# nabeelscicom/DistilCodec_nabeel

Measured on AMD Instinct MI355X. Metric: 24 kHz samples/s encode+decode at 1/8 GPU; code-index bit-exact vs CPU, higher is better.
Workload: dtype f32

## Files before the change

### distilcodec_nabeel_amd/csrc/dcx_conv_common.h

```cpp
#pragma once
#include <algorithm>
#include <type_traits>

#include "dcx_kernels.h"
#include "dcx_planes.h"

namespace dcx {

typedef float f32x16 __attribute__((ext_vector_type(16)));
typedef float f32x4 __attribute__((ext_vector_type(4)));
typedef float f32x2 __attribute__((ext_vector_type(2)));
typedef short s16x8 __attribute__((ext_vector_type(8)));
typedef short s16x4 __attribute__((ext_vector_type(4)));
typedef __bf16 bf16x8 __attribute__((ext_vector_type(8)));

constexpr int BK = 16;
constexpr int LDSK = 20;
template <bool SWZ>
struct XRow {
  static constexpr int kStride = SWZ ? 48 : 56;
  __device__ static __forceinline__ int half(int row, int h) { return SWZ ? h ^ ((row >> 3) & 1) : h; }
  __device__ static __forceinline__ int off(int row, int piece) {
    const int h = piece >= 3;
    return row * kStride + (half(row, h) * 3 + piece - 3 * h) * 8;
  }
};

__device__ __forceinline__ float silu_f(float v) { return v * __builtin_amdgcn_rcpf(1.0f + __expf(-v)); }
__device__ __forceinline__ float gelu_f(float v) { return 0.5f * v * (1.0f + erff(v * 0.70710678118654752440f)); }
__device__ __forceinline__ float gelu_bf16_f(float v) {
#ifdef DCX_GELU_ERF
  return gelu_f(v);
#endif
  const float z = fabsf(v) * 0.70710678118654752440f;
  const float t = __builtin_amdgcn_rcpf(fmaf(0.5f, z, 1.0f));
  float q = 0.17087277f;
  q = fmaf(q, t, -0.82215223f);
  q = fmaf(q, t, 1.48851587f);
  q = fmaf(q, t, -1.13520398f);
  q = fmaf(q, t, 0.27886807f);
  q = fmaf(q, t, -0.18628806f);
  q = fmaf(q, t, 0.09678418f);
  q = fmaf(q, t, 0.37409196f);
  q = fmaf(q, t, 1.00002368f);
  const float c = t * __expf(fmaf(t, q, fmaf(-z, z, -1.26551223f)));
  const float e = v >= 0.0f ? 1.0f - c : c - 1.0f;
  return 0.5f * v * (1.0f + e);
}

__device__ __forceinline__ f32x2 gelu_bf16_f2(f32x2 v) {
#ifdef DCX_GELU_SCALAR
  return f32x2{gelu_bf16_f(v[0]), gelu_bf16_f(v[1])};
#endif
  const f32x2 z = __builtin_elementwise_abs(v) * 0.70710678118654752440f;
  const f32x2 d = __builtin_elementwise_fma(f32x2{0.5f, 0.5f}, z, f32x2{1.0f, 1.0f});
  const f32x2 t = {__builtin_amdgcn_rcpf(d[0]), __builtin_amdgcn_rcpf(d[1])};
  auto fm = [&](f32x2 q, float c) { return __builtin_elementwise_fma(q, t, f32x2{c, c}); };
  f32x2 q = {0.17087277f, 0.17087277f};
  q = fm(q, -0.82215223f);
  q = fm(q, 1.48851587f);
  q = fm(q, -1.13520398f);
  q = fm(q, 0.27886807f);
  q = fm(q, -0.18628806f);
  q = fm(q, 0.09678418f);
  q = fm(q, 0.37409196f);
  q = fm(q, 1.00002368f);
  const f32x2 arg = __builtin_elementwise_fma(t, q, __builtin_elementwise_fma(-z, z, f32x2{-1.26551223f, -1.26551223f}));
  const f32x2 c = t * f32x2{__expf(arg[0]), __expf(arg[1])};
  const f32x2 e = {v[0] >= 0.0f ? 1.0f - c[0] : c[0] - 1.0f, v[1] >= 0.0f ? 1.0f - c[1] : c[1] - 1.0f};
  return 0.5f * v * (1.0f + e);
}

__device__ __forceinline__ int xcd_remap(int bid, int nwg) {
  const int xcd = bid & 7, q = nwg >> 3, r = nwg & 7;
  return (xcd < r ? xcd * (q + 1) : r * (q + 1) + (xcd - r) * q) + (bid >> 3);
}

__device__ __forceinline__ void flat_tile(int tpc, int batch, int& wg, int& b, int& ph) {
  const int t = xcd_remap(blockIdx.x, gridDim.x);
  const int per_ph = tpc * batch;
  ph = t / per_ph;
  const int r = t - ph * per_ph;
  b = r / tpc;
  wg = r - b * tpc;
}

__device__ __forceinline__ void ksplit_slice(const ConvParams& p, int b, int& clip, int& c0, int& nchunks) {
  clip = b;
  c0 = 0;
  nchunks = p.Cin / BK;
  if (p.ksplit > 1) {
    const int clips = p.batch / p.ksplit, sl = b / clips;
    clip = b - sl * clips;
    const int nunits = nchunks / p.kunit, base = nunits / p.ksplit, extra = nunits % p.ksplit;
    c0 = (sl * base + min(sl, extra)) * p.kunit;
    nchunks = (base + (sl < extra ? 1 : 0)) * p.kunit;
  }
}

static __device__ __attribute__((used, aligned(16))) float g_zero_row[32] = {0.f};

#if defined(DCX_CLOCK_DIAG) || defined(DCX_SEG_DIAG) || defined(DCX_TILE_DIAG)
#define DCX_DIAG 1
constexpr int kTileDiagMax = 16384;
[[maybe_unused]] static __device__ unsigned long long g_clock_diag[3], g_seg_diag[13], g_seg_diag8[49];
[[maybe_unused]] static __device__ unsigned long long g_tile_diag[kTileDiagMax * 6];
[[maybe_unused]] static __device__ unsigned int g_tile_cnt;
enum DiagSet : int { DIAG_CLOCK, DIAG_SEG, DIAG_SEG8, DIAG_TILES };
static int diag_read(int set, unsigned long long* out, int n, int reset) {
  if (set == DIAG_TILES) {
    unsigned int cnt = 0;
    if (hipMemcpyFromSymbol(&cnt, HIP_SYMBOL(g_tile_cnt), sizeof cnt) != hipSuccess) return -1;
    cnt = std::min(cnt, (unsigned)std::max(0, std::min(n, kTileDiagMax)));
    if (cnt && hipMemcpyFromSymbol(out, HIP_SYMBOL(g_tile_diag), sizeof(unsigned long long) * 6 * cnt) != hipSuccess) return -1;
    const unsigned int z = 0;
    if (reset && hipMemcpyToSymbol(HIP_SYMBOL(g_tile_cnt), &z, sizeof z) != hipSuccess) return -1;
    return (int)cnt;
  }
  const void* sym = set == DIAG_CLOCK ? (const void*)g_clock_diag : set == DIAG_SEG ? (const void*)g_seg_diag : (const void*)g_seg_diag8;
  unsigned long long v[49] = {};
  if (n > 49 || hipMemcpyFromSymbol(v, sym, sizeof(unsigned long long) * n) != hipSuccess) return -1;
  for (int i = 0; i < n; ++i) out[i] += v[i];
  const unsigned long long z[49] = {};
  if (reset && hipMemcpyToSymbol(sym, z, sizeof(unsigned long long) * n) != hipSuccess) return -1;
  return 0;
}
#define DCX_DIAG_FILE(tag) \
  int diag_##tag(int set, unsigned long long* out, int n, int reset) { return diag_read(set, out, n, reset); }
#else
#define DCX_DIAG_FILE(tag)
#endif
#ifdef DCX_SEG_DIAG
#define DCX_SEGT(v) const unsigned long long v = __builtin_amdgcn_s_memtime()
#else
#define DCX_SEGT(v)
#endif
#ifdef DCX_TILE_DIAG
#define DCX_TILET(v) const unsigned long long v = __builtin_amdgcn_s_memrealtime()
#else
#define DCX_TILET(v)
#endif

struct EpiPre {
  int osh;
  float acur;
  bool track;
};
template <int RROW>
__device__ __forceinline__ EpiPre epi_range_pre(const ConvParams& p, const ConvParams& pr, int b) {
  EpiPre e{0, 0.f, false};
  const bool h2o = (p.y6 && p.y_layout == LAYOUT_H2) || (p.y6s && p.ys_layout != LAYOUT_PLANES);
  const bool h2row = (RROW & 2) && h2o && pr.yb.rowwise;
  if (h2o && !h2row) {
    const float bnd = range_bound(pr.yb, b);
    e.osh = __builtin_amdgcn_readfirstlane(h2_shift(bnd));
    if (threadIdx.x == 0) {
      if (pr.y_ash) pr.y_ash[b] = e.osh;
      if (pr.rflag && !(bnd <= 3.0e38f)) atomicOr(pr.rflag, RANGE_NONFINITE);
    }
  }
  const bool track = pr.y_amax != nullptr;
  e.track = track;
  e.acur = track && !h2row ? __builtin_bit_cast(float, __builtin_amdgcn_readfirstlane(
                                                           __builtin_bit_cast(int, range_cur(pr.y_amax, b))))
                           : 0.f;
  return e;
}

struct EpiGeneric {
  static constexpr bool fixed = false;
};
template <int EPI, int MEAN, bool Y, bool Y2, bool Y6H, bool Y6SH, bool TRACK, bool ROWWISE = false>
struct EpiForm {
  static constexpr bool fixed = true;
  static constexpr int epi = EPI, mean = MEAN;
  static constexpr bool y = Y, y2 = Y2, y6h = Y6H, y6sh = Y6SH, track = TRACK, rowwise = ROWWISE;
};
template <typename F>
inline bool epi_form_is(const ConvParams& p) {
  const bool h2o = F::y6h || F::y6sh;
  return p.epi == F::epi && p.mean_mode == F::mean && !p.round_bf16 && (p.y != nullptr) == F::y &&
         (p.y2 != nullptr) == F::y2 && (p.y6 != nullptr) == F::y6h && (p.y6s != nullptr) == F::y6sh &&
         (!p.y6 || p.y_layout == LAYOUT_H2) && (!p.y6s || p.ys_layout == LAYOUT_H2) && (p.y_amax != nullptr) == F::track &&
         (h2o ? (p.yb.rowwise != 0) == F::rowwise : true) && (F::epi != EPI_GELU || p.w6 != nullptr) &&
         (F::mean == MEAN_NONE || p.macc != nullptr);
}

template <int BM, int BN, int WM, int WN, int LDS_FLOATS, int NT, int RROW, bool RAG, typename F, typename AccT>
__device__ __forceinline__ void epilogue_form(const ConvParams& p, const ConvParams& pr, AccT& acc, int q0, int co0, int b,
                                              int ph, float* smem, const EpiPre& pre) {
  constexpr int WR = BM / WM, WC = BN / WN;
  static_assert(sizeof(acc[0][0]) == 16 && sizeof(acc) == WR * WC * 4 / 64, "16 x 16 accumulator blocks");
  constexpr int LDSW = BN + 4;
  constexpr int RPP = (BM * LDSW <= LDS_FLOATS) ? BM
                      : (BM / 2 * LDSW <= LDS_FLOATS) ? BM / 2
                      : (BM / 4 * LDSW <= LDS_FLOATS) ? BM / 4 : WR;
  static_assert(RPP % WR == 0 && RPP * LDSW <= LDS_FLOATS, "epilogue pass does not fit LDS");
  const int tid = threadIdx.x, lane = tid & 63, wave = tid >> 6;
  const int wm = wave / WN, wn = wave % WN;
  const long long ob = (long long)b * p.y_bstride;
  constexpr bool RIN = RROW & 1, ROUT = RROW & 2;
  constexpr bool h2o = F::y6h || F::y6sh, h2row = ROUT && h2o && F::rowwise;
  constexpr bool need_r = F::epi == EPI_GAMMA_RES || F::epi == EPI_RES;
  constexpr bool need_m = F::mean == MEAN_MID || F::mean == MEAN_LAST;
  static_assert(!((F::mean == MEAN_FIRST || F::mean == MEAN_MID) && (F::y || F::y2 || h2o || F::track)), "mean form");
  unsigned short* const y6 = F::y6h ? p.y6 + ob * 2 : nullptr;
  unsigned short* const y6s = F::y6sh ? p.y6s + ob * 2 : nullptr;
  const float osc = __builtin_bit_cast(
      float, __builtin_amdgcn_readfirstlane(__builtin_bit_cast(int, __builtin_ldexpf(1.0f, h2o && !h2row ? pre.osh : 0))));
  float vmax = 0.f;
  const int lq_live = RAG ? clip_rows(pr.clip_len, pr.len_mul, b, p.Lq) : p.Lq;
  constexpr int G = 8, NH = 2;
  static_assert(NT % (BN / G) == 0, "each thread keeps one channel group");
  const int cg = (tid % (BN / G)) * G, trow = tid / (BN / G), co = co0 + cg;
  const int hsw = (lane >> 3) & 1;
  f32x4 bias4[NH], gamma4[NH];
#pragma unroll
  for (int h = 0; h < NH; ++h) {
    bias4[h] = p.bias ? *reinterpret_cast<const f32x4*>(p.bias + co + 4 * h) : f32x4{0.f, 0.f, 0.f, 0.f};
    gamma4[h] = F::epi == EPI_GAMMA_RES ? *reinterpret_cast<const f32x4*>(p.gamma + co + 4 * h) : f32x4{0.f, 0.f, 0.f, 0.f};
  }
  constexpr int RSTEP = NT / (BN / G), ROWS_T = RPP / RSTEP;
  static_assert(RPP % RSTEP == 0, "epilogue rows per thread");
  constexpr auto div_cap = [](int n, int cap) {
    int d = n < cap ? n : cap;
    while (n % d) --d;
    return d;
  };
  constexpr int IB = div_cap(ROWS_T, need_r || need_m ? 4 / NH : 8 / NH);
  auto row_bound = [&](int q) { return fmaf(pr.yb.g[0], fmaxf(pr.yb.m[0][(long long)b * p.Lq + q], pr.yb.f[0]), pr.yb.c); };

  auto pass = [&](int r0, auto fullt) {
    constexpr bool FULL = decltype(fullt)::value;
    f32x4 r[IB][NH], m[IB][NH];
    float rin[RIN ? IB : 1], rbnd[h2row ? IB : 1];
    auto load = [&](int rb) {
#pragma unroll
      for (int k = 0; k < IB; ++k) {
        const int qq = q0 + r0 + trow + (rb + k) * RSTEP;
        const int q = FULL ? qq : min(qq, p.Lq - 1);
        const long long o = ob + ((long long)q * p.out_mul + ph) * p.ldy + co;
#pragma unroll
        for (int h = 0; h < NH; ++h) {
          if constexpr (need_r) r[k][h] = *reinterpret_cast<const f32x4*>(p.res + o + 4 * h);
          if constexpr (need_m) m[k][h] = *reinterpret_cast<const f32x4*>(p.macc + o + 4 * h);
        }
        if constexpr (RIN) rin[k] = pr.x_ash_row ? __builtin_ldexpf(1.0f, -pr.x_ash_row[(long long)b * p.Lin + q]) : 1.0f;
        if constexpr (h2row) rbnd[k] = row_bound(q);
      }
    };
    load(0);
    __syncthreads();
    if (wm * WR >= r0 && wm * WR < r0 + RPP) {
#pragma unroll
      for (int i = 0; i < WR / 16; ++i)
#pragma unroll
        for (int j = 0; j < WC / 16; ++j)
#pragma unroll
          for (int e = 0; e < 4; ++e) {
            const int row = wm * WR + i * 16 + 4 * (lane >> 4) + e - r0;
            smem[row * LDSW + wn * WC + j * 16 + (lane & 15)] = acc[i][j][e];
          }
    }
    __syncthreads();
#pragma unroll
    for (int rb = 0; rb < ROWS_T; rb += IB) {
      f32x4 x[IB][NH];
      float rsc[IB];
#pragma unroll
      for (int k = 0; k < IB; ++k) {
        const int rl = trow + (rb + k) * RSTEP;
        const int q = q0 + r0 + rl;
        const bool dead = RAG && q >= lq_live;
        const float rin_ = RIN ? rin[RIN ? k : 0] : 1.0f;
        const f32x4 u = *reinterpret_cast<const f32x4*>(smem + rl * LDSW + cg + 4 * hsw);
        const f32x4 v = *reinterpret_cast<const f32x4*>(smem + rl * LDSW + cg + 4 * (1 - hsw));
        x[k][0] = (hsw ? v : u) * rin_ + bias4[0];
        x[k][1] = (hsw ? u : v) * rin_ + bias4[1];
#pragma unroll
        for (int h = 0; h < NH; ++h) {
          if constexpr (F::epi == EPI_GELU) {
#pragma unroll
            for (int e = 0; e < 4; e += 2) {
              const f32x2 g = gelu_bf16_f2(f32x2{x[k][h][e], x[k][h][e + 1]});
              x[k][h][e] = g[0];
              x[k][h][e + 1] = g[1];
            }
          } else if constexpr (F::epi == EPI_GAMMA_RES) {
            x[k][h] = r[k][h] + gamma4[h] * x[k][h];
          } else if constexpr (F::epi == EPI_RES) {
            x[k][h] = r[k][h] + x[k][h];
          } else {
            static_assert(F::epi == EPI_BIAS, "epilogue form");
          }
          if (dead) x[k][h] = f32x4{0.f, 0.f, 0.f, 0.f};
          if constexpr (F::mean == MEAN_MID) x[k][h] = dead ? x[k][h] : m[k][h] + x[k][h];
          if constexpr (F::mean == MEAN_LAST) x[k][h] = dead ? x[k][h] : (m[k][h] + x[k][h]) / 3.0f;
        }
        rsc[k] = osc;
        if constexpr (h2row) rsc[k] = rbnd[k];
      }
      if (rb + IB < ROWS_T) load(rb + IB);
#pragma unroll
      for (int k = 0; k < IB; ++k) {
        const int q = q0 + r0 + trow + (rb + k) * RSTEP;
        if (!FULL && q >= p.Lq) continue;
        const long long orow = (long long)q * p.out_mul + ph;
        const long long o = ob + orow * p.ldy + co;
        if constexpr (F::mean == MEAN_FIRST || F::mean == MEAN_MID) {
#pragma unroll
          for (int h = 0; h < NH; ++h) *reinterpret_cast<f32x4*>(p.macc + o + 4 * h) = x[k][h];
          continue;
        }
        float sc = rsc[k];
        if constexpr (h2row) {
          const float bnd = rsc[k];
          const int sh = h2_shift(bnd);
          sc = __builtin_ldexpf(1.0f, sh);
          if (cg == 0 && pr.y_ash) pr.y_ash[(long long)b * p.Lq + q] = sh;
          if (pr.rflag && !(bnd <= 3.0e38f)) atomicOr(pr.rflag, RANGE_NONFINITE);
        }
        if constexpr (F::track) {
          const float ts = h2row ? sc : 1.0f;
#pragma unroll
          for (int h = 0; h < NH; ++h)
#pragma unroll
            for (int e = 0; e < 4; ++e) vmax = fmaxf(vmax, fabsf(x[k][h][e]) * ts);
        }
        if constexpr (F::y) {
#pragma unroll
          for (int h = 0; h < NH; ++h) *reinterpret_cast<f32x4*>(p.y + o + 4 * h) = x[k][h];
        }
        float xv[8];
#pragma unroll
        for (int e = 0; e < 8; ++e) xv[e] = x[k][e >> 2][e & 3];
        if constexpr (F::y6h) store_h2_8<false>(y6, orow, p.Cout, co, xv, sc);
        if constexpr (F::y2 || F::y6sh) {
          float sv[8];
#pragma unroll
          for (int e = 0; e < 8; ++e) sv[e] = silu_f(xv[e]);
          if constexpr (F::y2) {
            *reinterpret_cast<f32x4*>(p.y2 + o) = f32x4{sv[0], sv[1], sv[2], sv[3]};
            *reinterpret_cast<f32x4*>(p.y2 + o + 4) = f32x4{sv[4], sv[5], sv[6], sv[7]};
          }
          if constexpr (F::y6sh) store_h2_8<false>(y6s, orow, p.Cout, co, sv, sc);
        }
      }
    }
  };
#pragma unroll 1
  for (int r0 = 0; r0 < BM; r0 += RPP) {
    if (q0 + r0 + RPP <= p.Lq) pass(r0, std::true_type{});
    else pass(r0, std::false_type{});
  }
  if constexpr (F::track)
    range_report_wg(vmax, h2row ? nullptr : pr.y_amax, b, h2row ? 65504.0f : h2o ? 65504.0f / osc : __builtin_inff(),
                    pr.rflag, pre.acur, smem, NT);
}

template <int BM, int BN, int WM, int WN, int LDS_FLOATS, int NT, int RROW = 2, bool RAG = true, typename F = EpiGeneric,
          typename AccT>
__device__ __forceinline__ void epilogue_lds(const ConvParams& p, const ConvParams& pr, AccT& acc, int q0, int co0,
                                             int b, int ph, float* smem, const EpiPre* pre = nullptr) {
#ifndef DCX_EPI4
  if constexpr (F::fixed) {
    epilogue_form<BM, BN, WM, WN, LDS_FLOATS, NT, RROW, RAG, F>(p, pr, acc, q0, co0, b, ph, smem, *pre);
    return;
  }
#endif
  constexpr int WR = BM / WM, WC = BN / WN;
  constexpr int TM = WR / 32, TN = WC / 32;
  constexpr bool M16 = sizeof(acc[0][0]) == 16;
  static_assert(sizeof(acc) == WR * WC * 4 / 64, "accumulator tile");
  constexpr int LDSW = BN + 4;
  constexpr int RPP = (BM * LDSW <= LDS_FLOATS) ? BM
                      : (BM / 2 * LDSW <= LDS_FLOATS) ? BM / 2
                      : (BM / 4 * LDSW <= LDS_FLOATS) ? BM / 4 : WR;
  static_assert(RPP % WR == 0 && RPP * LDSW <= LDS_FLOATS, "epilogue pass does not fit LDS");
  const int tid = threadIdx.x, lane = tid & 63, wave = tid >> 6;
  const int wm = wave / WN, wn = wave % WN;
  const int lrow = lane & 31, rhalf = 4 * (lane >> 5);
  const long long ob = (long long)b * p.y_bstride;
  unsigned short* y6 = p.y6 ? p.y6 + ob * layout_u16(p.y_layout) : nullptr;
  unsigned short* y6s = p.y6s ? p.y6s + ob * (p.ys_layout != LAYOUT_PLANES ? 2 : 3) : nullptr;
  const bool h2o = (y6 && p.y_layout == LAYOUT_H2) || (y6s && p.ys_layout != LAYOUT_PLANES);
  constexpr bool RIN = RROW & 1, ROUT = RROW & 2;
  const bool h2row = ROUT && h2o && pr.yb.rowwise;
  int osh = 0;
  if (pre) {
    osh = pre->osh;
  } else if (h2o && !h2row) {
    const float bnd = range_bound(pr.yb, b);
    osh = __builtin_amdgcn_readfirstlane(h2_shift(bnd));
    if (tid == 0) {
      if (pr.y_ash) pr.y_ash[b] = osh;
      if (pr.rflag && !(bnd <= 3.0e38f)) atomicOr(pr.rflag, RANGE_NONFINITE);
    }
  }
// ... 160 lines not shown
          if (p.round_bf16) x[h] = round_bf16x4(x[h]);
        }
      }
      float rsc = osc;
      if (h2row) {
        const long long grow = (long long)b * p.Lq + q;
        const float bnd = RIN ? rbnd[RIN ? k : 0] : row_bound(q);
        const int sh = h2_shift(bnd);
        rsc = __builtin_ldexpf(1.0f, sh);
        if (cg == 0 && pr.y_ash) pr.y_ash[grow] = sh;
        if (pr.rflag && !(bnd <= 3.0e38f)) atomicOr(pr.rflag, RANGE_NONFINITE);
      }
      if (track) {
        const float ts = h2row ? rsc : 1.0f;
#pragma unroll
        for (int h = 0; h < NH; ++h)
#pragma unroll
          for (int e = 0; e < 4; ++e) vmax = fmaxf(vmax, fabsf(x[h][e]) * ts);
      }
      if (p.y) {
#pragma unroll
        for (int h = 0; h < NH; ++h) *reinterpret_cast<f32x4*>(p.y + o + 4 * h) = x[h];
      }
      if constexpr (G == 8) {
        float xv[8];
#pragma unroll
        for (int e = 0; e < 8; ++e) xv[e] = x[e >> 2][e & 3];
        if (y6) {
          if (p.y_layout == LAYOUT_BF16) store_bf16x8(y6, orow, p.Cout, co, xv);
          else if ((int)p.y_layout == 2) store_hm8(y6, orow, p.Cout, co, xv);
          else if (p.y_layout == LAYOUT_H2) store_h2_8<false>(y6, orow, p.Cout, co, xv, rsc);
          else store_planes8(y6, orow, p.Cout, co, xv);
        }
        if (p.y2 || y6s) {
          float sv[8];
#pragma unroll
          for (int e = 0; e < 8; ++e) sv[e] = p.round_bf16 ? bf16_val(bf16_bits(silu_f(xv[e]))) : silu_f(xv[e]);
          if (p.y2) {
            *reinterpret_cast<f32x4*>(p.y2 + o) = f32x4{sv[0], sv[1], sv[2], sv[3]};
            *reinterpret_cast<f32x4*>(p.y2 + o + 4) = f32x4{sv[4], sv[5], sv[6], sv[7]};
          }
          if (y6s) {
            if (p.ys_layout != LAYOUT_PLANES) store_h2_8<false>(y6s, orow, p.Cout, co, sv, rsc);
            else store_planes8(y6s, orow, p.Cout, co, sv);
          }
        }
      } else {
        if (y6) {
          if (p.y_layout == LAYOUT_BF16) store_bf16x4(y6, orow, p.Cout, co, x[0][0], x[0][1], x[0][2], x[0][3]);
          else if ((int)p.y_layout == 2) store_hm4(y6, orow, p.Cout, co, x[0][0], x[0][1], x[0][2], x[0][3]);
          else if (p.y_layout == LAYOUT_H2) store_h2_4<false>(y6, orow, p.Cout, co, x[0][0], x[0][1], x[0][2], x[0][3], rsc);
          else store_planes4(y6, orow, p.Cout, co, x[0][0], x[0][1], x[0][2], x[0][3]);
        }
        if (p.y2 || y6s) {
          f32x4 sv;
#pragma unroll
          for (int e = 0; e < 4; ++e) sv[e] = p.round_bf16 ? bf16_val(bf16_bits(silu_f(x[0][e]))) : silu_f(x[0][e]);
          if (p.y2) *reinterpret_cast<f32x4*>(p.y2 + o) = sv;
          if (y6s) {
            if (p.ys_layout != LAYOUT_PLANES) store_h2_4<false>(y6s, orow, p.Cout, co, sv[0], sv[1], sv[2], sv[3], rsc);
            else store_planes4(y6s, orow, p.Cout, co, sv[0], sv[1], sv[2], sv[3]);
          }
        }
      }
    }
  };
  constexpr int IBF0 = 8 / NH, IBM0 = 4 / NH;
  constexpr auto div_cap = [](int n, int cap) {
    int d = n < cap ? n : cap;
    while (n % d) --d;
    return d;
  };
  constexpr int IBF = div_cap(ROWS_T, IBF0), IBM = div_cap(ROWS_T, IBM0);
  static_assert(ROWS_T % IBF == 0 && ROWS_T % IBM == 0, "epilogue batches");
#pragma unroll 1
  for (int r0 = 0; r0 < BM; r0 += RPP) {
    if (need_m) {
#pragma unroll
      for (int rb = 0; rb < ROWS_T; rb += IBM) batch(r0, rb, rb == 0, std::integral_constant<int, IBM>{});
    } else {
#pragma unroll
      for (int rb = 0; rb < ROWS_T; rb += IBF) batch(r0, rb, rb == 0, std::integral_constant<int, IBF>{});
    }
  }
  if (track)
    range_report_wg(vmax, h2row ? nullptr : pr.y_amax, b, h2row ? 65504.0f : h2o ? 65504.0f / osc : __builtin_inff(),
                    pr.rflag, acur, smem, NT);
}

__device__ __forceinline__ bool tile_dead(const ConvParams& p, const ConvParams& pr, int b, int q0) {
  return pr.clip_len != nullptr && q0 >= clip_rows(pr.clip_len, pr.len_mul, b, p.Lq);
}
template <int BM, int BN, int NT>
__device__ __forceinline__ void epilogue_dead(const ConvParams& p, const ConvParams& pr, int q0, int co0, int b, int ph) {
  const long long ob = (long long)b * p.y_bstride;
  unsigned short* y6 = p.y6 ? p.y6 + ob * layout_u16(p.y_layout) : nullptr;
  unsigned short* y6s = p.y6s ? p.y6s + ob * (p.ys_layout != LAYOUT_PLANES ? 2 : 3) : nullptr;
  const bool h2o = (y6 && p.y_layout == LAYOUT_H2) || (y6s && p.ys_layout != LAYOUT_PLANES);
  if (h2o && threadIdx.x == 0) {
    const float bnd = range_bound(pr.yb, b);
    if (pr.y_ash) pr.y_ash[b] = h2_shift(bnd);
    if (pr.rflag && !(bnd <= 3.0e38f)) atomicOr(pr.rflag, RANGE_NONFINITE);
  }
  const f32x4 z4 = {0.f, 0.f, 0.f, 0.f};
  const float z8[8] = {0.f, 0.f, 0.f, 0.f, 0.f, 0.f, 0.f, 0.f};
  constexpr int CG = BN / 8;
  for (int i = threadIdx.x; i < BM * CG; i += NT) {
    const int q = q0 + i / CG, co = co0 + (i % CG) * 8;
    if (q >= p.Lq) break;
    const long long orow = (long long)q * p.out_mul + ph;
    const long long o = ob + orow * p.ldy + co;
    if (p.mean_mode == MEAN_FIRST || p.mean_mode == MEAN_MID) {
      *reinterpret_cast<f32x4*>(p.macc + o) = z4;
      *reinterpret_cast<f32x4*>(p.macc + o + 4) = z4;
      continue;
    }
    if (p.y) {
      *reinterpret_cast<f32x4*>(p.y + o) = z4;
      *reinterpret_cast<f32x4*>(p.y + o + 4) = z4;
    }
    if (y6) {
      if (p.y_layout == LAYOUT_BF16) store_bf16x8(y6, orow, p.Cout, co, z8);
      else if (p.y_layout == LAYOUT_H2) store_h2_8<false>(y6, orow, p.Cout, co, z8, 1.0f);
      else store_planes8(y6, orow, p.Cout, co, z8);
    }
    if (p.y2) {
      *reinterpret_cast<f32x4*>(p.y2 + o) = z4;
      *reinterpret_cast<f32x4*>(p.y2 + o + 4) = z4;
    }
    if (y6s) {
      if (p.ys_layout != LAYOUT_PLANES) store_h2_8<false>(y6s, orow, p.Cout, co, z8, 1.0f);
      else store_planes8(y6s, orow, p.Cout, co, z8);
    }
  }
}

typedef __attribute__((address_space(3))) void* lds_ptr_t;

__device__ __forceinline__ void dma16(__amdgpu_buffer_rsrc_t r, unsigned short* lds, int voff, int soff) {
  __builtin_amdgcn_raw_ptr_buffer_load_lds(r, (lds_ptr_t)lds, 16, voff, soff, 0, 0);
}
__device__ __forceinline__ void seg_barrier() { asm volatile("s_waitcnt lgkmcnt(0)\n\ts_barrier" ::: "memory"); }
__device__ __forceinline__ void wait_dma(int n) {
#define DCX_W(k) \
  case k: asm volatile("s_waitcnt vmcnt(" #k ")" ::: "memory"); break;
  switch (n) {
    DCX_W(1) DCX_W(2) DCX_W(3) DCX_W(4) DCX_W(5) DCX_W(6) DCX_W(7) DCX_W(8) DCX_W(9) DCX_W(10) DCX_W(11)
    DCX_W(12) DCX_W(13) DCX_W(14) DCX_W(15) DCX_W(16) DCX_W(17) DCX_W(18) DCX_W(19) DCX_W(20) DCX_W(21) DCX_W(22)
    DCX_W(23)
    default: asm volatile("s_waitcnt vmcnt(0)" ::: "memory");
  }
#undef DCX_W
}

}
```

### distilcodec_nabeel_amd/csrc/dcx_conv_h3.hip

```cpp
#include <atomic>

#include "dcx_conv_common.h"
#include "dcx_conv_launch.h"
#include "dcx_conv_pingpong.h"
#include "dcx_a3_layout.h"
#include "dcx_w3_layout.h"

namespace dcx {

DCX_DIAG_FILE(h3)

typedef _Float16 f16x8 __attribute__((ext_vector_type(8)));

using EpiC1 = EpiForm<EPI_BIAS, MEAN_NONE, false, false, false, true, true>;
using EpiUp = EpiForm<EPI_BIAS, MEAN_NONE, true, false, false, true, true>;
using EpiC2 = EpiForm<EPI_RES, MEAN_NONE, true, false, false, true, true>;
using EpiMeanF = EpiForm<EPI_RES, MEAN_FIRST, false, false, false, false, false>;
using EpiMeanM = EpiForm<EPI_RES, MEAN_MID, false, false, false, false, false>;
using EpiMeanLH = EpiForm<EPI_RES, MEAN_LAST, false, false, false, true, true>;
using EpiMeanLF = EpiForm<EPI_RES, MEAN_LAST, false, true, false, false, true>;
using EpiPw1 = EpiForm<EPI_GELU, MEAN_NONE, false, false, true, false, false, true>;
using EpiPw2 = EpiForm<EPI_GAMMA_RES, MEAN_NONE, true, false, false, false, false>;

static std::atomic<long long> g_form_launches[kEpiFormCounters];
// ... 220 lines not shown
  auto dmaB1 = [&](int c, int m, int slot, int i) {
#ifdef DCX_X3_NODMA
    if (in_loop) return;
#endif
    const int k = (group ? B_G0 : 0) + i * 4 + gw;
    dma16(rw, lds + NA * ABUF / 2 + slot * (BBUF / 2) + k * 512, b_lane, w3_step_bytes(nchunks, p.Cout, m, c) + w3_wide_piece(BN, k));
  };
  auto dma_step = [&](int c, int m, int slot) {
    if (m == 0) {
#pragma unroll
      for (int i = 0; i < A_PW; ++i) dmaA1(c, slot, i);
    }
#pragma unroll
    for (int i = 0; i < B_W0; ++i) dmaB1(c, m, slot, i);
  };
  auto dma_step1 = [&](int c, int m, int slot) {
#pragma unroll
    for (int i = 0; i < B_W1; ++i) dmaB1(c, m, slot, i);
  };

  const int l15 = lane & 15, kg = lane >> 4;
  const char* const ldsb = reinterpret_cast<const char*>(lds);
  const int a_row = wm * WR + l15;
  static_assert(WR % kA3BlockRows == 0 && a3_image(16, 0) == 2048, "row blocks as immediates");
  const char* const b_rd = ldsb + NA * ABUF + kg * BN * 16 + (wn * WC + l15) * 16;
  s16x8 aq[TM][2], bq[TN][2];
  auto readF = [&](int c, int m, int slot) {
    const int a_r = a_row + (HALO ? m * p.in_step - lo_rel : 0);
    const int ah = (HALO ? (c & 1) : slot) * ABUF + (ROWS ? a3_image(a_r, kg) : kg * AR * 16 + a_r * 16);
    const char* a = ldsb + ah;
    const char* al = ldsb + (ROWS ? ah ^ kA3PlaneXor : ah + 4 * AR * 16);
    const char* bb = b_rd + slot * BBUF;
#pragma unroll
    for (int j = 0; j < TN; ++j) {
      bq[j][0] = *reinterpret_cast<const s16x8*>(bb + j * 256);
      bq[j][1] = *reinterpret_cast<const s16x8*>(bb + j * 256 + 4 * BN * 16);
    }
#pragma unroll
    for (int i = 0; i < TM; ++i) {
      aq[i][0] = *reinterpret_cast<const s16x8*>(a + i * (ROWS ? 2048 : 256));
      aq[i][1] = *reinterpret_cast<const s16x8*>(al + i * (ROWS ? 2048 : 256));
    }
  };
  f32x4 acc[TM][TN];
  zero_acc(acc);
  auto mfma = [&]() {
    __builtin_amdgcn_s_setprio(1);
#pragma unroll
    for (int k = 0; k < 3; ++k) {
      const int sa = k == 1 ? 1 : 0, sb = k == 0 ? 1 : 0;
#pragma unroll
      for (int i = 0; i < TM; ++i) {
#pragma unroll
        for (int j = 0; j < TN; ++j)
          acc[i][j] = __builtin_amdgcn_mfma_f32_16x16x32_f16(__builtin_bit_cast(f16x8, aq[i][sa]),
                                                             __builtin_bit_cast(f16x8, bq[j][sb]), acc[i][j], 0, 0, 0);
      }
    }
    __builtin_amdgcn_s_setprio(0);
  };

  int cl = 0, ml = 0;
  if (SPLIT && tid == 0) *rd_cnt = 0u;
  for (int t = 0; t < 2 && t < nsteps; ++t) {
    if (group == 0) dma_step(cl, ml, t);
    else if (SPLIT) dma_step1(cl, ml, t);
    step_adv(cl, ml, taps);
  }
  const EpiPre epre = epi_range_pre<HALO == 0 ? 3 : 0>(p, pr, b);
  const float unscale = __builtin_bit_cast(float, __builtin_amdgcn_readfirstlane(__builtin_bit_cast(int,
      __builtin_ldexpf(1.0f, -(p.w3_shift + (pr.x_ash ? pr.x_ash[b] : pr.x_ash_c))))));
  asm volatile("s_waitcnt vmcnt(0)" ::: "memory");
  seg_barrier();
  DCX_TILET(tile_t1);
  in_loop = true;
#ifdef DCX_SEG_DIAG
  unsigned long long sd[6] = {};
#endif
  int cr = 0, mr = 0;
  if (group == 0) {
    readF(0, 0, 0);
    if (SPLIT) {
      asm volatile("s_waitcnt lgkmcnt(0)" ::: "memory");
      if (lane == 0) __hip_atomic_fetch_add(rd_cnt, 1u, __ATOMIC_RELAXED, __HIP_MEMORY_SCOPE_WORKGROUP);
    }
    step_adv(cr, mr, taps);
    for (int s = 0; s < nsteps; ++s) {
      DCX_SEGT(ta);
      mfma();
      asm volatile("s_waitcnt vmcnt(0)" ::: "memory");
      DCX_SEGT(tb);
      seg_barrier();
      DCX_SEGT(tc);
      if (s + 2 < nsteps) {
        dma_step(cl, ml, s & 1);
        step_adv(cl, ml, taps);
      }
      DCX_SEGT(tr);
      if (s + 1 < nsteps) readF(cr, mr, (s + 1) & 1);
      DCX_SEGT(tq);
      DCX_SEGT(td);
      seg_barrier();
      DCX_SEGT(te);
#ifdef DCX_SEG_DIAG
      sd[0] += tb - ta; sd[1] += tc - tb; sd[2] += td - tc; sd[3] += te - td; sd[4] += tr - tc; sd[5] += tq - tr;
#endif
      step_adv(cr, mr, taps);
    }
  } else {
    for (int s = 0; s < nsteps; ++s) {
      DCX_SEGT(ta);
      readF(cr, mr, s & 1);
      if (SPLIT) {
        int n = 0;
        if (s + 2 < nsteps) {
          asm volatile("s_waitcnt lgkmcnt(0)" ::: "memory");
          if (lane == 0) __hip_atomic_fetch_add(rd_cnt, 1u, __ATOMIC_RELAXED, __HIP_MEMORY_SCOPE_WORKGROUP);
          const unsigned int want = 4u * (unsigned)(s + 2);
          while (__hip_atomic_load(rd_cnt, __ATOMIC_RELAXED, __HIP_MEMORY_SCOPE_WORKGROUP) < want) {
          }
          dma_step1(cl, ml, s & 1);
          step_adv(cl, ml, taps);
          n = B_W1;
        }
        wait_dma(n);
      }
      DCX_SEGT(tb);
      seg_barrier();
      DCX_SEGT(tc);
      mfma();
      DCX_SEGT(td);
      seg_barrier();
      DCX_SEGT(te);
#ifdef DCX_SEG_DIAG
      sd[2] += tb - ta; sd[3] += tc - tb; sd[0] += td - tc; sd[1] += te - td; sd[5] += tb - ta;
#endif
      step_adv(cr, mr, taps);
    }
  }
#ifdef DCX_SEG_DIAG
  if ((threadIdx.x & 255) == 0) {
#pragma unroll
    for (int i = 0; i < 6; ++i) atomicAdd(&g_seg_diag[group * 6 + i], sd[i]);
    if (group == 0) atomicAdd(&g_seg_diag[12], (unsigned long long)nsteps);
  }
  if (lane == 0) {
#pragma unroll
    for (int i = 0; i < 6; ++i) atomicAdd(&g_seg_diag8[wave * 6 + i], sd[i]);
    if (wave == 0) atomicAdd(&g_seg_diag8[48], (unsigned long long)nsteps);
  }
#endif
  asm volatile("s_waitcnt vmcnt(0)" ::: "memory");
  DCX_TILET(tile_t2);
#pragma unroll
  for (int i = 0; i < TM; ++i)
#pragma unroll
    for (int j = 0; j < TN; ++j) acc[i][j] *= unscale;
  epilogue_lds<BM, BN, WM, WN, LDS_B / 4, 512, HALO == 0 ? 3 : 0, RAG, F>(p, pr, acc, q0, co0, b, ph, reinterpret_cast<float*>(lds), &epre);
  DCX_TILE_END(nsteps);
}

template <int HALO, bool SPLIT, int BN = 256, bool RAG = false, typename F = EpiGeneric>
__global__ void __launch_bounds__(512, 2) conv_gemm_x3dw(const ConvParams p) {
  constexpr int BM = BN == 256 ? 256 : 384;
  int wg, b, ph;
  flat_tile(((p.Lq + BM - 1) / BM) * (p.Cout / BN), p.batch, wg, b, ph);
  x3dw_tile<HALO, SPLIT, BN, RAG, false, F>(p, p, wg, b, ph);
}

template <bool SPLIT, int BN = 256, bool RAG = false, typename F = EpiGeneric>
__global__ void __launch_bounds__(512, 2) conv_gemm_x3dw_group(const ConvGroup g) {
  ConvParams p;
  int local, b;
  const ConvParams& pr = group_member(g, p, local, b);
  x3dw_tile<64, SPLIT, BN, RAG, true, F>(p, pr, local, b, 0);
}

bool x3dq_ok(const ConvParams& p, int bn, bool wide) {
  const int span = (p.taps - 1) * (p.in_step < 0 ? -p.in_step : p.in_step);
  if (!p.x6 || !p.w3 || p.x_layout != LAYOUT_H2 || p.Cin % 32 || p.Cout % bn || p.ksplit > 1) return false;
  const long long arow = (long long)p.ldx * 4;
  if ((long long)p.taps * p.Cin * p.Cout * 4 >= (1LL << 31)) return false;
  if (p.taps == 1) {
    for (int i = 0; i < kMaxPhases; ++i)
      if (p.in_base[i] < 0) return false;
    return 256LL * arow < (1LL << 31);
  }
  return p.taps >= (wide ? 2 : 3) && span > 0 && span <= 64 && (long long)(p.Lin + 1024) * arow < (1LL << 31);
}
int x3dq_bn(const ConvParams& p) {
  const int k = p.kn ? p.kn->h3_bn : 0;
  if (p.Cout % 256) return (k == 128 && p.taps >= 3) || p.taps < 2 ? 128 : 384;
  if (p.taps == 2) return 512;
  return k == 128 ? 128 : k == 256 ? 256 : 512;
}

template <int BN>
hipError_t launch_x3dq(const ConvParams& p, int batch, int phases, hipStream_t s, const char** kname) {
  constexpr int BM = 32768 / BN;
  if (p.taps == 1) {
    if (p.clip_len) return hipErrorNotSupported;
    if (kname) *kname = BN == 256 ? "conv_gemm_x3dm<128,256>" : "conv_gemm_x3dm<256,128>";
    return launch_flat<BM, BN>(conv_gemm_x3dq<BN, 0>, p, batch, phases, 512, s);
  }
  if (kname) *kname = BN == 256 ? "conv_gemm_x3dq<128,256,halo>" : "conv_gemm_x3dq<256,128,halo>";
  if (p.clip_len) return launch_flat<BM, BN>(conv_gemm_x3dq<BN, 64, true>, p, batch, phases, 512, s);
  return launch_flat<BM, BN>(conv_gemm_x3dq<BN, 64>, p, batch, phases, 512, s);
}

template hipError_t launch_x3dq<256>(const ConvParams&, int, int, hipStream_t, const char**);
template hipError_t launch_x3dq<128>(const ConvParams&, int, int, hipStream_t, const char**);

template <int BM, int BN, bool RAG>
static hipError_t launch_x3dw_halo(const ConvParams& p, bool sp, int batch, int phases, hipStream_t s) {
  if (!sp) {
    ++g_form_launches[kEpiFormCounters - 1];
    return launch_flat<BM, BN>(conv_gemm_x3dw<64, false, BN, RAG>, p, batch, phases, 512, s);
  }
  return with_epi_form<EpiC1, EpiUp, EpiC2, EpiMeanF, EpiMeanM, EpiMeanLH, EpiMeanLF>(p, knobs(p).epi_generic, [&](auto f) {
    return launch_flat<BM, BN>(conv_gemm_x3dw<64, true, BN, RAG, decltype(f)>, p, batch, phases, 512, s);
  });
}

hipError_t launch_x3dw(const ConvParams& p, int bsel, int batch, int phases, hipStream_t s, const char** kname) {
  const bool sp = knobs(p).h3_split;
  if (p.clip_len && p.taps == 1) return hipErrorNotSupported;
  if (bsel == 384) {
    if (kname) *kname = "conv_gemm_x3dw<384,128,halo>";
    return p.clip_len ? launch_x3dw_halo<384, 128, true>(p, sp, batch, phases, s)
                      : launch_x3dw_halo<384, 128, false>(p, sp, batch, phases, s);
  }
  if (p.taps == 1) {
    if (kname) *kname = "conv_gemm_x3dw<256,256>";
    if (!sp) {
      ++g_form_launches[kEpiFormCounters - 1];
      return launch_flat<256, 256>(conv_gemm_x3dw<0, false>, p, batch, phases, 512, s);
    }
    return with_epi_form<EpiPw1, EpiPw2>(p, knobs(p).epi_generic, [&](auto f) {
      return launch_flat<256, 256>(conv_gemm_x3dw<0, true, 256, false, decltype(f)>, p, batch, phases, 512, s);
    });
  }
  if (kname) *kname = "conv_gemm_x3dw<256,256,halo>";
  return p.clip_len ? launch_x3dw_halo<256, 256, true>(p, sp, batch, phases, s)
                    : launch_x3dw_halo<256, 256, false>(p, sp, batch, phases, s);
}

template <int BN, bool RAG>
static void launch_x3dw_group(const ConvGroup& g, bool split, unsigned blocks, hipStream_t s) {
  if (!split) {
    ++g_form_launches[kEpiFormCounters - 1];
    hipLaunchKernelGGL((conv_gemm_x3dw_group<false, BN, RAG>), dim3(blocks), dim3(512), 0, s, g);
    return;
  }
  (void)with_epi_form<EpiC1, EpiC2>(g.p[0], group_generic(g), [&](auto f) {
    hipLaunchKernelGGL((conv_gemm_x3dw_group<true, BN, RAG, decltype(f)>), dim3(blocks), dim3(512), 0, s, g);
    return hipSuccess;
  });
}

hipError_t launch_h3_group(const ConvGroup& g, int bsel, bool split, unsigned blocks, hipStream_t s, const char** kname) {
  const bool rag = g.p[0].clip_len != nullptr;
  if (bsel == 384) {
    if (kname) *kname = "conv_gemm_x3dw_group<384,128,halo>";
    if (rag) launch_x3dw_group<128, true>(g, split, blocks, s);
    else launch_x3dw_group<128, false>(g, split, blocks, s);
  } else if (bsel == 512) {
    if (kname) *kname = "conv_gemm_x3dw_group<256,256,halo>";
    if (rag) launch_x3dw_group<256, true>(g, split, blocks, s);
    else launch_x3dw_group<256, false>(g, split, blocks, s);
  } else if (bsel == 256) {
    if (kname) *kname = "conv_gemm_x3dq_group<128,256,halo>";
    if (rag) hipLaunchKernelGGL((conv_gemm_x3dq_group<256, true>), dim3(blocks), dim3(512), 0, s, g);
    else hipLaunchKernelGGL((conv_gemm_x3dq_group<256>), dim3(blocks), dim3(512), 0, s, g);
  } else {
    if (kname) *kname = "conv_gemm_x3dq_group<256,128,halo>";
    if (rag) hipLaunchKernelGGL((conv_gemm_x3dq_group<128, true>), dim3(blocks), dim3(512), 0, s, g);
    else hipLaunchKernelGGL((conv_gemm_x3dq_group<128>), dim3(blocks), dim3(512), 0, s, g);
  }
  return hipGetLastError();
}

}
```

Before: 52.45 million.

## Stream residual and bias into LDS ring via buffer DMA in conv epilogue

Adds a triple-buffered LDS ring for the fixed-form residual epilogue of the x3dw conv kernel. Residual rows and the bias are prefetched with buffer_load_lds DMA, two passes ahead, and overlap the accumulator dumps and stores through explicit vmcnt waits. This replaces the per-thread global residual loads that followed a barrier in the old epilogue. The cost is more LDS use, intricate wait-count bookkeeping and a narrower set of epilogue forms that take the path. It also adds a debug macro that skips the epilogue loads.

Result: no change. 52.68 million (median of 6 runs) (+0.5%).

```diff
diff --git a/distilcodec_nabeel_amd/csrc/dcx_conv_common.h b/distilcodec_nabeel_amd/csrc/dcx_conv_common.h
--- a/distilcodec_nabeel_amd/csrc/dcx_conv_common.h
+++ b/distilcodec_nabeel_amd/csrc/dcx_conv_common.h
@@ -2,6 +2,7 @@
 #include <algorithm>
 #include <type_traits>
 
+#include "dcx_epi_ring.h"
 #include "dcx_kernels.h"
 #include "dcx_planes.h"
 
@@ -242,8 +243,13 @@
         const long long o = ob + ((long long)q * p.out_mul + ph) * p.ldy + co;
 #pragma unroll
         for (int h = 0; h < NH; ++h) {
+#ifdef DCX_EPI_NOLOAD
+          (void)o;
+          r[k][h] = m[k][h] = f32x4{0.f, 0.f, 0.f, 0.f};
+#else
           if constexpr (need_r) r[k][h] = *reinterpret_cast<const f32x4*>(p.res + o + 4 * h);
           if constexpr (need_m) m[k][h] = *reinterpret_cast<const f32x4*>(p.macc + o + 4 * h);
+#endif
         }
         if constexpr (RIN) rin[k] = pr.x_ash_row ? __builtin_ldexpf(1.0f, -pr.x_ash_row[(long long)b * p.Lin + q]) : 1.0f;
         if constexpr (h2row) rbnd[k] = row_bound(q);
@@ -710,5 +716,190 @@
   }
 #undef DCX_W
 }
-
-}
+template <int N>
+__device__ __forceinline__ void wait_vm() {
+  asm volatile("s_waitcnt vmcnt(%0)" ::"n"(N) : "memory");
+}
+
+template <typename F>
+constexpr bool epi_ring_form() {
+#ifndef DCX_EPI4
+  if constexpr (F::fixed) return F::epi == EPI_RES && (F::mean == MEAN_NONE || F::mean == MEAN_FIRST);
+#endif
+  return false;
+}
+
+template <int BM, int BN>
+struct EpiRingDma {
+  __amdgpu_buffer_rsrc_t rres;
+  int lane_off, rowb, wave;
+  char* lds;
+  __device__ __forceinline__ EpiRingDma(const ConvParams& p, int q0, int co0, int b, int ph, char* lds_) : lds(lds_) {
+    const int lane = threadIdx.x & 63;
+    wave = __builtin_amdgcn_readfirstlane(threadIdx.x >> 6);
+    rowb = p.out_mul * p.ldy * 4;
+    const int live = min(p.Lq - q0, BM);
+    const float* base = p.res + (long long)b * p.y_bstride + ((long long)q0 * p.out_mul + ph) * p.ldy + co0;
+    rres = __builtin_amdgcn_make_buffer_rsrc((void*)base, 0, (live - 1) * rowb + BN * 4, 0x00020000);
+    lane_off = epi_ring_lane_row(BN, lane) * rowb + epi_ring_lane_col(BN, lane);
+  }
+  __device__ __forceinline__ void issue(int i, int slot) const {
+    constexpr int P = epi_ring_pass(BN), RPI = epi_ring_rows_inst(BN);
+#pragma unroll
+    for (int k = 0; k < kEpiRingInst / 8; ++k) {
+      const int j = wave * (kEpiRingInst / 8) + k;
+      dma16(rres, reinterpret_cast<unsigned short*>(lds + epi_ring_buf(BN, 0) + slot * kEpiRingBuf + j * 1024),
+            lane_off + (i * P + j * RPI) * rowb, 0);
+    }
+  }
+  __device__ __forceinline__ void burst(const ConvParams& p, int co0) const {
+    if (wave == 0) {
+      const __amdgpu_buffer_rsrc_t rb =
+          __builtin_amdgcn_make_buffer_rsrc((void*)(p.bias ? p.bias + co0 : nullptr), 0, p.bias ? BN * 4 : 0, 0x00020000);
+      dma16(rb, reinterpret_cast<unsigned short*>(lds + epi_ring_bias(BN)), (int)(threadIdx.x & 63) * 16, 0);
+    }
+    issue(0, 0);
+    issue(1, 1);
+  }
+};
+
+template <int BM, int BN, int WM, int WN, int NT, bool RAG, typename F, typename AccT>
+__device__ __forceinline__ void epilogue_ring(const ConvParams& p, const ConvParams& pr, AccT& acc, const EpiRingDma<BM, BN>& dma,
+                                              int q0, int co0, int b, int ph, char* lds, const EpiPre& pre) {
+  constexpr int WR = BM / WM, WC = BN / WN, TM = WR / 16, TN = WC / 16;
+  static_assert(sizeof(acc[0][0]) == 16 && sizeof(acc) == WR * WC * 4 / 64, "16 x 16 accumulator blocks");
+  constexpr int P = epi_ring_pass(BN), NP = BM / P, D = kEpiRingDepth, LDSW = BN + 4;
+  constexpr int G = 8, NH = 2, RSTEP = NT / (BN / G), IB = P / RSTEP;
+  static_assert(NT == 512 && BM % P == 0 && P % 16 == 0 && IB == 2 && NP >= 3, "pass shape");
+  static_assert(epi_ring_form<F>() && !F::y6h && !F::rowwise, "ring form");
+  constexpr bool macc_only = F::mean == MEAN_FIRST;
+  static_assert(!(macc_only && (F::y || F::y2 || F::y6sh || F::track)), "mean form");
+  constexpr int S = IB * (macc_only ? NH : (F::y ? NH : 0) + (F::y2 ? NH : 0) + (F::y6sh ? 2 : 0));
+  static_assert(2 * S + 8 < 64, "vmcnt");
+  const int tid = threadIdx.x, lane = tid & 63, wave = dma.wave;
+  const int wm = wave / WN, wn = wave % WN;
+  const long long ob = (long long)b * p.y_bstride;
+  unsigned short* const y6s = F::y6sh ? p.y6s + ob * 2 : nullptr;
+  const float osc = __builtin_bit_cast(
+      float, __builtin_amdgcn_readfirstlane(__builtin_bit_cast(int, __builtin_ldexpf(1.0f, F::y6sh ? pre.osh : 0))));
+  float vmax = 0.f;
+  const int lq_live = RAG ? clip_rows(pr.clip_len, pr.len_mul, b, p.Lq) : p.Lq;
+  const int cg = (tid % (BN / G)) * G, trow = tid / (BN / G), co = co0 + cg;
+  const int hsw = (lane >> 3) & 1;
+  float* const smem = reinterpret_cast<float*>(lds);
+  const char* const bias_l = lds + epi_ring_bias(BN) + cg * 4;
+
+  auto rows = [&](int r0, int slot, auto fullt) {
+    constexpr bool FULL = decltype(fullt)::value;
+    const char* const rbuf = lds + epi_ring_buf(BN, 0) + slot * kEpiRingBuf;
+    f32x4 x[IB][NH];
+    const f32x4 bu = *reinterpret_cast<const f32x4*>(bias_l + 16 * hsw);
+    const f32x4 bv = *reinterpret_cast<const f32x4*>(bias_l + 16 * (1 - hsw));
+    const f32x4 bias4[NH] = {hsw ? bv : bu, hsw ? bu : bv};
+#pragma unroll
+    for (int k = 0; k < IB; ++k) {
+      const int rl = trow + k * RSTEP;
+      const int q = q0 + r0 + rl;
+      const bool dead = RAG && q >= lq_live;
+      const f32x4 u = *reinterpret_cast<const f32x4*>(smem + rl * LDSW + cg + 4 * hsw);
+      const f32x4 v = *reinterpret_cast<const f32x4*>(smem + rl * LDSW + cg + 4 * (1 - hsw));
+      const f32x4 ru = *reinterpret_cast<const f32x4*>(rbuf + epi_ring_image(BN, rl, cg + 4 * hsw));
+      const f32x4 rv = *reinterpret_cast<const f32x4*>(rbuf + epi_ring_image(BN, rl, cg + 4 * (1 - hsw)));
+      x[k][0] = (hsw ? v : u) + bias4[0];
+      x[k][1] = (hsw ? u : v) + bias4[1];
+      x[k][0] = (hsw ? rv : ru) + x[k][0];
+      x[k][1] = (hsw ? ru : rv) + x[k][1];
+#pragma unroll
+      for (int h = 0; h < NH; ++h)
+        if (dead) x[k][h] = f32x4{0.f, 0.f, 0.f, 0.f};
+    }
+#pragma unroll
+    for (int k = 0; k < IB; ++k) {
+      const int q = q0 + r0 + trow + k * RSTEP;
+      if (!FULL && q >= p.Lq) continue;
+      const long long orow = (long long)q * p.out_mul + ph;
+      const long long o = ob + orow * p.ldy + co;
+      if constexpr (macc_only) {
+#pragma unroll
+        for (int h = 0; h < NH; ++h) *reinterpret_cast<f32x4*>(p.macc + o + 4 * h) = x[k][h];
+        continue;
+      }
+      if constexpr (F::track) {
+#pragma unroll
+        for (int h = 0; h < NH; ++h)
+#pragma unroll
+          for (int e = 0; e < 4; ++e) vmax = fmaxf(vmax, fabsf(x[k][h][e]) * 1.0f);
+      }
+      if constexpr (F::y) {
+#pragma unroll
+        for (int h = 0; h < NH; ++h) *reinterpret_cast<f32x4*>(p.y + o + 4 * h) = x[k][h];
+      }
+      if constexpr (F::y2 || F::y6sh) {
+        float sv[8];
+#pragma unroll
+        for (int e = 0; e < 8; ++e) sv[e] = silu_f(x[k][e >> 2][e & 3]);
+        if constexpr (F::y2) {
+          *reinterpret_cast<f32x4*>(p.y2 + o) = f32x4{sv[0], sv[1], sv[2], sv[3]};
+          *reinterpret_cast<f32x4*>(p.y2 + o + 4) = f32x4{sv[4], sv[5], sv[6], sv[7]};
+        }
+        if constexpr (F::y6sh) store_h2_8<false>(y6s, orow, p.Cout, co, sv, osc);
+      }
+    }
+  };
+  auto dump_block = [&](auto it, int t) {
+    constexpr int I = decltype(it)::value;
+#pragma unroll
+    for (int j = 0; j < TN; ++j)
+#pragma unroll
+      for (int e = 0; e < 4; ++e)
+        smem[(t * 16 + 4 * (lane >> 4) + e) * LDSW + wn * WC + j * 16 + (lane & 15)] = acc[I][j][e];
+  };
+
+  const int np_live = min(NP, (p.Lq - q0 + P - 1) / P);
+  int slot = 0, slot2 = 2;
+#pragma unroll 1
+  for (int i = 0; i < np_live; ++i) {
+    const int r0 = i * P;
+    const bool full = q0 + r0 + P <= p.Lq;
+    seg_barrier();
+    if (i + 2 < NP) dma.issue(i + 2, slot2);
+#pragma unroll
+    for (int t = 0; t < P / 16; ++t) {
+      const int gb = r0 / 16 + t;
+      if (wm == gb / TM) {
+        const int I = gb % TM;
+        if (I == 0) dump_block(std::integral_constant<int, 0>{}, t);
+        if (I == 1) dump_block(std::integral_constant<int, 1>{}, t);
+        if (I == 2) dump_block(std::integral_constant<int, 2>{}, t);
+        if constexpr (TM > 3)
+          if (I == 3) dump_block(std::integral_constant<int, 3>{}, t);
+      }
+    }
+    if (full) {
+      const int a = min(2, NP - 1 - i), c = min(2, i);
+      switch (a * 3 + c) {
+        case 0: wait_vm<0>(); break;
+        case 1: wait_vm<S>(); break;
+        case 2: wait_vm<2 * S>(); break;
+        case 3: wait_vm<4>(); break;
+        case 4: wait_vm<4 + S>(); break;
+        case 5: wait_vm<4 + 2 * S>(); break;
+        case 6: wait_vm<8>(); break;
+        case 7: wait_vm<8 + S>(); break;
+        default: wait_vm<8 + 2 * S>(); break;
+      }
+    } else {
+      wait_vm<0>();
+    }
+    seg_barrier();
+    if (full) rows(r0, slot, std::true_type{});
+    else rows(r0, slot, std::false_type{});
+    slot = slot == D - 1 ? 0 : slot + 1;
+    slot2 = slot2 == D - 1 ? 0 : slot2 + 1;
+  }
+  if (np_live < NP) wait_vm<0>();
+  if constexpr (F::track)
+    range_report_wg(vmax, pr.y_amax, b, F::y6sh ? 65504.0f / osc : __builtin_inff(), pr.rflag, pre.acur, smem, NT);
+}
+
+}
diff --git a/distilcodec_nabeel_amd/csrc/dcx_conv_h3.hip b/distilcodec_nabeel_amd/csrc/dcx_conv_h3.hip
--- a/distilcodec_nabeel_amd/csrc/dcx_conv_h3.hip
+++ b/distilcodec_nabeel_amd/csrc/dcx_conv_h3.hip
@@ -396,11 +396,23 @@
 #endif
   asm volatile("s_waitcnt vmcnt(0)" ::: "memory");
   DCX_TILET(tile_t2);
-#pragma unroll
-  for (int i = 0; i < TM; ++i)
-#pragma unroll
-    for (int j = 0; j < TN; ++j) acc[i][j] *= unscale;
-  epilogue_lds<BM, BN, WM, WN, LDS_B / 4, 512, HALO == 0 ? 3 : 0, RAG, F>(p, pr, acc, q0, co0, b, ph, reinterpret_cast<float*>(lds), &epre);
+  constexpr bool RING = HALO != 0 && epi_ring_form<F>();
+  auto unscale_acc = [&]() {
+#pragma unroll
+    for (int i = 0; i < TM; ++i)
+#pragma unroll
+      for (int j = 0; j < TN; ++j) acc[i][j] *= unscale;
+  };
+  if constexpr (RING) {
+    static_assert(epi_ring_bytes(BN) <= LDS_B, "the epilogue ring lies inside the tile's LDS");
+    const EpiRingDma<BM, BN> rdma(p, q0, co0, b, ph, reinterpret_cast<char*>(lds));
+    rdma.burst(p, co0);
+    unscale_acc();
+    epilogue_ring<BM, BN, WM, WN, 512, RAG, F>(p, pr, acc, rdma, q0, co0, b, ph, reinterpret_cast<char*>(lds), epre);
+  } else {
+    unscale_acc();
+    epilogue_lds<BM, BN, WM, WN, LDS_B / 4, 512, HALO == 0 ? 3 : 0, RAG, F>(p, pr, acc, q0, co0, b, ph, reinterpret_cast<float*>(lds), &epre);
+  }
   DCX_TILE_END(nsteps);
 }
 
diff --git a/distilcodec_nabeel_amd/csrc/dcx_epi_ring.h b/distilcodec_nabeel_amd/csrc/dcx_epi_ring.h
--- /dev/null
+++ b/distilcodec_nabeel_amd/csrc/dcx_epi_ring.h
@@ -0,0 +1,20 @@
+#pragma once
+
+namespace dcx {
+
+constexpr int kEpiRingDepth = 3;
+constexpr int kEpiRingBuf = 32 * 1024;
+constexpr int kEpiRingInst = 32;
+constexpr int kEpiRingLdsMax = 160 * 1024;
+
+constexpr int epi_ring_pass(int bn) { return kEpiRingBuf / (bn * 4); }
+constexpr int epi_ring_stage(int bn) { return epi_ring_pass(bn) * (bn + 4) * 4; }
+constexpr int epi_ring_buf(int bn, int slot) { return epi_ring_stage(bn) + slot * kEpiRingBuf; }
+constexpr int epi_ring_bias(int bn) { return epi_ring_buf(bn, kEpiRingDepth); }
+constexpr int epi_ring_bytes(int bn) { return epi_ring_bias(bn) + 1024; }
+constexpr int epi_ring_rows_inst(int bn) { return 1024 / (bn * 4); }
+constexpr int epi_ring_lane_row(int bn, int lane) { return lane / (bn / 4); }
+constexpr int epi_ring_lane_col(int bn, int lane) { return lane % (bn / 4) * 16; }
+constexpr int epi_ring_image(int bn, int row, int col) { return (row * bn + col) * 4; }
+
+}
```
